# iSEE-Laboratory/DiffuVolume

Hardware: AMD Instinct MI355X
Metric: stereo pairs/sec, SceneFlow 960x540 (cropped 960x512) maxdisp=192, hot path (higher is better)
Workload: dtype f32; 1 GPU; SceneFlow ACVNet+DiffuVolume hot path (gwc + concat*softmax(att) + 5 DDIM steps + EPE), 960x512, maxdisp=192, batch=8/GPU, random-init weights; global_batch=8, ddim_steps=5, parallelism=dp1

## Files before the change

### diffuvolume_amd/_lib.py

```python
from __future__ import annotations

import ctypes
import os
from ctypes import POINTER, Structure, c_char_p, c_double, c_float, c_int, c_size_t, c_void_p
from pathlib import Path

import torch

_LIB_PATH = Path(os.environ.get("DV_LIB_PATH") or Path(__file__).resolve().parent / "libdiffuvolume_hip.so")
_lib = None


class DvDdimCoef(Structure):
    _fields_ = [("sqrt_recip_alpha", c_double), ("sqrt_recipm1_alpha", c_double),
                ("sqrt_alpha_next", c_double), ("c", c_double), ("sigma", c_double),
                ("dif_thr", c_float), ("unc_thr", c_float), ("cof", c_float), ("last", c_int),
                ("clamp_max", c_float), ("ens_dif_thr", c_float)]


P = c_void_p
I = c_int
SIGNATURES = {
    "dv_version": (c_int, []),
    "dv_error_string": (c_char_p, [I]),
# ... 4 lines not shown
    "dv_pointwise_expand_packed_floats": (c_size_t, [I, I]),
    "dv_pointwise_expand_pack_weights_f32": (c_int, [P, P, I, I, P]),
    "dv_pointwise_expand_f32": (c_int, [P, P, P, I, I, I, I, P]),
    "dv_softmax_d_f32": (c_int, [P, P, I, I, I, P]),
    "dv_mul_f32": (c_int, [P, P, P, c_size_t, P]),
    "dv_conv3d_rank1_filter_f32": (c_int, [P, P, P, P, P, P, I, I, I, I, I, I, P]),
    "dv_noise_prepare_f32": (c_int, [P, P, P, I, I, I, P]),
    "dv_noise_prepare_f64": (c_int, [P, P, P, P, I, I, I, P]),
    "dv_conv3d_packed_floats": (c_size_t, [I, I, I]),
    "dv_conv3d_pack_weights_f32": (c_int, [P, P, I, I, I, P]),
    "dv_conv3d_f32": (c_int, [P, P, P, P, P, P, P, I, I, I, I, I, I, I, I, I, P]),
    "dv_conv3d_set_s2_tile": (c_int, [I]),
    "dv_conv3d_set_c1z": (c_int, [I, I]),
    "dv_conv3d_f16x3_packed_bytes": (c_size_t, [I, I]),
    "dv_conv3d_f16x3_pack_weights": (c_int, [P, P, I, I, P]),
    "dv_conv3d_f16x3_f32": (c_int, [P, P, P, P, P, P, P, P, I, I, I, I, I, I, I, P]),
    "dv_conv3d_wino_packed_floats": (c_size_t, [I, I]),
    "dv_conv3d_wino_pack_weights_f32": (c_int, [P, P, I, I, P]),
    "dv_conv3d_wino_f32": (c_int, [P, P, P, P, P, P, P, I, I, I, I, I, I, I, P]),
    "dv_conv3d_wino3_packed_floats": (c_size_t, [I, I]),
    "dv_conv3d_wino3_supported": (c_int, [I, I, I, I, I]),
    "dv_conv3d_wino3_pack_weights_f32": (c_int, [P, P, I, I, P]),
    "dv_conv3d_wino3_f32": (c_int, [P, P, P, P, P, P, I, I, I, I, I, I, I, P]),
    "dv_conv3d_s2pp_supported": (c_int, [I, I, I, I, I]),
    "dv_conv3d_s2pp_packed_floats": (c_size_t, [I, I]),
    "dv_conv3d_s2pp_pack_weights_f32": (c_int, [P, P, I, I, P]),
    "dv_conv3d_s2pp_f32": (c_int, [P, P, P, P, P, P, I, I, I, I, I, I, I, P]),
    "dv_deconv3d_packed_floats": (c_size_t, [I, I]),
    "dv_deconv3d_pack_weights_f32": (c_int, [P, P, I, I, P]),
    "dv_deconv3d_k3s2_f32": (c_int, [P, P, P, P, P, P, I, I, I, I, I, I, I, P]),
    "dv_deconv3d_pl_supported": (c_int, [I, I, I, I, I, I]),
    "dv_deconv3d_set_impl": (c_int, [I]),
    "dv_deconv3d_pl_set_max_blocks": (c_int, [I]),
    "dv_deconv3d_k4_packed_floats": (c_size_t, [I, I]),
    "dv_deconv3d_k4_pack_weights_f32": (c_int, [P, P, I, I, P]),
    "dv_deconv3d_k4s2_f32": (c_int, [P, P, P, P, P, P, I, I, I, I, I, I, I, P]),
    "dv_conv2d_packed_floats": (c_size_t, [I, I, I, I]),
    "dv_conv2d_pack_weights_f32": (c_int, [P, P, I, I, I, I, P]),
    "dv_conv2d_f32": (c_int, [P, P, P, P, P, P, I, I, I, I, I, I, I, I, P]),
    "dv_conv2d_gated_f32": (c_int, [P, P, P, P, P, P, P, P, P, I, I, I, I, I, I, I, I, P]),
    "dv_conv2d_cat_f32": (c_int, [P, P, I, P, P, P, P, P, P, P, P, I, I, I, I, I, I, I, P]),
    "dv_conv2d_auto_kslices": (c_int, [I, I, I, I, I, I, I]),
    "dv_conv2d_cat_ksplit_f32": (c_int, [P, P, I, P, P, P, P, P, P, P, P, P, I, I, I, I, I, I, I, I, P]),
    "dv_conv2d_s2_f32": (c_int, [P, P, P, P, P, P, I, I, I, I, I, I, I, P]),
    "dv_conv2d_wino_packed_floats": (c_size_t, [I, I]),
    "dv_conv2d_wino_pack_weights_f32": (c_int, [P, P, I, I, P]),
    "dv_conv2d_wino_cat_f32": (c_int, [P, P, I, P, P, P, P, P, P, P, P, I, I, I, I, I, P]),
    "dv_conv2d_wino_cat_pair_f32": (c_int, [P, P, I, P, P, P, P, P, P, P, P, P, I, I, I, I, I, I, P]),
    "dv_conv2d_wino_dil_cat_f32": (c_int, [P, P, I, P, P, P, P, P, P, P, P, I, I, I, I, I, I, P]),
    "dv_refine_inputs_f32": (c_int, [P, P, P, P, P, P, I, I, I, I, I, P]),
    "dv_space_to_batch2_f32": (c_int, [P, P, I, I, I, I, P]),
    "dv_conv2d_wino_auto_kslices": (c_int, [I, I, I, I, I]),
    "dv_conv2d_wino_cat_ksplit_f32": (c_int, [P, P, I, P, P, P, P, P, P, P, P, P, I, I, I, I, I, I, I, P]),
    "dv_conv2d_wino_cat_pair_ksplit_f32": (c_int, [P, P, I, P, P, P, P, P, P, P, P, P, P, I, I, I, I, I, I, I, P]),
    "dv_conv2d_wino_s2b_f32": (c_int, [P, P, I, P, P, P, P, I, I, I, I, I, P]),
    "dv_batch_to_space_f32": (c_int, [P, P, I, I, I, I, I, P]),
    "dv_softmax_regress_f32": (c_int, [P, P, I, I, I, I, P]),
    "dv_feature_gate_f32": (c_int, [P, P, P, I, I, I, I, I, P]),
    "dv_deconv3d_k3s2_redir_f32": (c_int, [P, P, P, P, P, P, I, I, I, I, I, I, I, I, P]),
    "dv_patch_volume_f32": (c_int, [P, P, P, P, P, I, I, I, I, I, P]),
    "dv_patch_volume_runs_f32": (c_int, [P, P, P, P, P, I, I, I, I, I, I, P, P, P, P]),
    "dv_window_attn3d_f32": (c_int, [P, P, P, P, P, P, I, I, I, I, I, I, P]),
    "dv_upsample_softmax_regress_f32": (c_int, [P, P, P, I, I, I, I, I, P]),
    "dv_upsample_softmax_uncertainty_f32": (c_int, [P, P, P, I, I, I, I, I, P]),
    "dv_disparity_regression_f32": (c_int, [P, P, I, I, I, I, P]),
    "dv_encode_two_hot_f32": (c_int, [P, P, I, I, I, P]),
# ... 88 lines not shown
```

### diffuvolume_amd/csrc/deconv3d.hip

```cpp
#include <atomic>
#include <type_traits>

#include "dv_common.h"

int dv_deconv3d_pl_run(const float* in, const float* wpacked, const float* ch_scale, const float* ch_bias, const float* residual,
                       const float* skip, const float* rw, float* out, int B, int Cin, int D, int H, int W, int Cout, int Cskip,
                       int act, size_t wpk_floats, hipStream_t s);

namespace {

std::atomic<int> g_deconv_impl_pin{0};

typedef float f32x4 __attribute__((ext_vector_type(4)));

constexpr int kTD = 2, kTH = 2, kMTX = 2, kNT = 2;
constexpr int kTW = kMTX * 16;
constexpr int kCOUT = kNT * 16;

template <int K, int KC_>
struct DGeo {
  static constexpr int KC = KC_;
  static constexpr int LO = (K == 4) ? 1 : 0;
  static constexpr int T = K * K * K;
  static constexpr int IZ = kTD + 1 + LO, IY = kTH + 1 + LO, IX = kTW + 1 + LO;
  static constexpr int PRAW = IZ * IY * IX;
  static constexpr int P = PRAW + ((16 - PRAW % 32) + 32) % 32;
  static constexpr int IN_FLOATS = KC * P, W_FLOATS = T * KC * kCOUT;
  static_assert(P % 32 == 16, "bank rule");
  static_assert((IN_FLOATS + W_FLOATS) * 4 <= 80 * 1024, "two blocks per CU");
};
__host__ __device__ constexpr int tap_par(int k) { return (k + 1) & 1; }
__host__ __device__ constexpr int tap_off(int k) { return (k == 0 ? 1 : 0) - (k == 3 ? 1 : 0); }

struct DeconvArgs {
  const float* in;
  const float* wpk;
  const float* ch_scale;
  const float* ch_bias;
  const float* residual;
  const float* skip;
  const float* rw;
  int Cskip;
  float* out;
  int B, Cin, D, H, W, Cout, Coutp;
// ... 382 lines not shown
  if (blocks <= 0 || blocks > 0x7fffffffLL) return DV_ERR_SHAPE;
  hipLaunchKernelGGL((deconv3d_mfma_kernel<K, KC_>), dim3((unsigned)blocks), dim3(256), 0, s, a);
  return dv_launch_status();
}

constexpr int kc_of(int K) { return K == 3 ? 8 : 4; }

int pack_any(const float* w, float* wpacked, int Cin, int Cout, int K, hipStream_t s) {
  const int T = K * K * K, KC = kc_of(K), nchunk = pad_to(Cin, 8) / KC, nco = pad_to(Cout, kCOUT) / kCOUT;
  const size_t total = (size_t)nchunk * nco * T * KC * kCOUT;
  const int blocks = (int)((total + 255) / 256 < 4096 ? (total + 255) / 256 : 4096);
  hipLaunchKernelGGL(pack_deconv_weights_kernel, dim3(blocks), dim3(256), 0, s, w, wpacked, Cin, Cout, nchunk, nco, T, KC);
  return dv_launch_status();
}

int run_any(const float* in, const float* wpacked, const float* ch_scale, const float* ch_bias,
            const float* residual, float* out, int B, int Cin, int D, int H, int W, int Cout, int act, int K,
            hipStream_t s, const float* skip = nullptr, const float* rw = nullptr, int Cskip = 0) {
  DeconvArgs a;
  a.skip = skip; a.rw = rw; a.Cskip = Cskip;
  a.in = in; a.wpk = wpacked; a.ch_scale = ch_scale; a.ch_bias = ch_bias; a.residual = residual;
  a.out = out; a.B = B; a.Cin = Cin; a.D = D; a.H = H; a.W = W; a.Cout = Cout;
  a.Coutp = pad_to(Cout, kCOUT);
  a.ntx = (W + kTW - 1) / kTW;
  a.nty = (H + kTH - 1) / kTH;
  a.ntz = (D + kTD - 1) / kTD;
  a.nco = a.Coutp / kCOUT;
  a.act = act;
  a.vec_store = (W % 4 == 0) && dv_aligned16(out) && (!residual || dv_aligned16(residual));
  if ((size_t)D * H * W * sizeof(float) > 0x7fffffffull) return DV_ERR_SHAPE;
  a.fast_ok = (W % 2 == 0) && dv_aligned16(out) && (!residual || dv_aligned16(residual)) &&
              (size_t)Cout * 8 * D * H * W * sizeof(float) <= 0xffffffffull;
  const int pin = g_deconv_impl_pin.load(std::memory_order_relaxed);
  if (K == 3 && pin != 1 && (pin == 2 || !residual) &&
      dv_deconv3d_pl_supported(Cin, Cout, D, H, W, skip ? Cskip : 0) && dv_aligned16(in) && dv_aligned16(out) &&
      (!residual || dv_aligned16(residual)) && (!skip || dv_aligned16(skip)))
    return dv_deconv3d_pl_run(in, wpacked, ch_scale, ch_bias, residual, skip, rw, out, B, Cin, D, H, W, Cout, Cskip, act,
                              dv_deconv3d_packed_floats(Cin, Cout), s);
  return K == 3 ? launch_deconv<3, 8>(a, s) : launch_deconv<4, 4>(a, s);
}

}

extern "C" int dv_deconv3d_set_impl(int mode) {
  DV_REQUIRE(mode >= 0 && mode <= 2, DV_ERR_UNSUPPORTED);
  g_deconv_impl_pin.store(mode, std::memory_order_relaxed);
  return DV_OK;
}

extern "C" size_t dv_deconv3d_packed_floats(int Cin, int Cout) {
  if (Cin <= 0 || Cout <= 0) return 0;
  return (size_t)pad_to(Cin, 8) * 27 * pad_to(Cout, kCOUT);
}

extern "C" size_t dv_deconv3d_k4_packed_floats(int Cin, int Cout) {
  if (Cin <= 0 || Cout <= 0) return 0;
  return (size_t)pad_to(Cin, 8) * 64 * pad_to(Cout, kCOUT);
}

extern "C" int dv_deconv3d_pack_weights_f32(const float* w, float* wpacked, int Cin, int Cout, dv_stream_t stream) {
  DV_REQUIRE_PTR(w);
  DV_REQUIRE_PTR(wpacked);
  DV_REQUIRE(Cin > 0 && Cout > 0, DV_ERR_SHAPE);
  return pack_any(w, wpacked, Cin, Cout, 3, (hipStream_t)stream);
}

extern "C" int dv_deconv3d_k4_pack_weights_f32(const float* w, float* wpacked, int Cin, int Cout, dv_stream_t stream) {
  DV_REQUIRE_PTR(w);
  DV_REQUIRE_PTR(wpacked);
  DV_REQUIRE(Cin > 0 && Cout > 0, DV_ERR_SHAPE);
  return pack_any(w, wpacked, Cin, Cout, 4, (hipStream_t)stream);
}

#define DV_DECONV_CHECKS                                                             \
  DV_REQUIRE_PTR(in);                                                                \
  DV_REQUIRE_PTR(wpacked);                                                           \
  DV_REQUIRE_PTR(out);                                                               \
  DV_REQUIRE(B > 0 && Cin > 0 && D > 0 && H > 0 && W > 0 && Cout > 0, DV_ERR_SHAPE);  \
  DV_REQUIRE(act >= DV_ACT_NONE && act <= DV_ACT_LEAKY, DV_ERR_UNSUPPORTED);         \
  DV_REQUIRE(dv_aligned16(wpacked), DV_ERR_ALIGN);
// ... 31 lines not shown
```

### diffuvolume_amd/csrc/deconv3d_pl.hip

```cpp
#include <atomic>
#include <type_traits>

#include "dv_common.h"

namespace {

std::atomic<int> g_pl_max_blocks{0};

typedef float f32x4 __attribute__((ext_vector_type(4)));
typedef float f32x2 __attribute__((ext_vector_type(2)));
typedef int i32x4 __attribute__((ext_vector_type(4)));

namespace pl {
constexpr int TH = 2, TW = 32, KC = 8, NT = 2, COUT = 16 * NT;
constexpr int RQ = TW / 4 + 1;
constexpr int RS = 4 * RQ;
constexpr int IY = TH + 1, ROWS = 2 * IY;
constexpr int QPC = 60;
constexpr int CS = 4 * QPC;
static_assert(ROWS * RQ <= QPC && CS % 64 == 48, "brick image");
constexpr int BRICK_Q = KC * QPC;
constexpr int BRICK_P = (BRICK_Q + 63) / 64;
constexpr int BRICK_FLOATS = BRICK_P * 256;
constexpr int W_FLOATS = 27 * KC * COUT;
// ... 339 lines not shown

template <bool SKIP, bool RES, int AM>
int pl_launch(const PLArgs& a, hipStream_t s) {
  const int cap = g_pl_max_blocks.load(std::memory_order_relaxed);
  const long long slots = cap > 0 ? cap : pl_cu_count();
  const long long pairs = ((long long)a.nsp * a.nco + 1) / 2;
  const unsigned blocks = (unsigned)(pairs < slots ? pairs : slots);
  hipLaunchKernelGGL((deconv3d_pl_kernel<SKIP, RES, AM>), dim3(blocks), dim3(512 + 64 * pl::NL), 0, s, a);
  return dv_launch_status();
}

}

extern "C" int dv_deconv3d_pl_set_max_blocks(int n) {
  DV_REQUIRE(n >= 0, DV_ERR_SHAPE);
  g_pl_max_blocks.store(n, std::memory_order_relaxed);
  return DV_OK;
}

extern "C" int dv_deconv3d_pl_supported(int Cin, int Cout, int D, int H, int W, int Cskip) {
  if (Cin <= 0 || Cout <= 0 || D <= 0 || H <= 0 || W <= 0 || Cskip < 0) return 0;
  if (Cin % pl::KC || Cout % pl::COUT || Cout > pl::MAXCO || W % 4) return 0;
  if (Cskip % pl::SKC || Cskip / pl::SKC > Cin / pl::KC) return 0;
  const size_t vol = (size_t)D * H * W;
  if (vol * sizeof(float) * pl::KC > 0x7fffffffull) return 0;
  if ((size_t)Cout * 8 * vol * sizeof(float) > 0xffffffffull) return 0;
  if ((size_t)Cskip * 8 * vol * sizeof(float) > 0xffffffffull) return 0;
  return 1;
}

int dv_deconv3d_pl_run(const float* in, const float* wpacked, const float* ch_scale, const float* ch_bias, const float* residual,
                       const float* skip, const float* rw, float* out, int B, int Cin, int D, int H, int W, int Cout, int Cskip,
                       int act, size_t wpk_floats, hipStream_t s) {
  PLArgs a;
  a.in = in; a.wpk = wpacked; a.ch_scale = ch_scale; a.ch_bias = ch_bias; a.residual = residual; a.skip = skip; a.rw = rw;
  a.out = out; a.B = B; a.Cin = Cin; a.D = D; a.H = H; a.W = W; a.Cout = Cout; a.Cskip = skip ? Cskip : 0; a.act = act;
  a.ntx = pl_cdiv(W, pl::TW); a.nty = pl_cdiv(H, pl::TH); a.nco = Cout / pl::COUT;
  const long long tiles = (long long)B * D * a.nty * a.ntx;
  if (tiles <= 0 || tiles * a.nco > 0x3fffffffLL) return DV_ERR_SHAPE;
  a.nsp = (int)tiles;
  if (wpk_floats * sizeof(float) > 0x7fffffffull) return DV_ERR_SHAPE;
  a.wpk_bytes = (unsigned)(wpk_floats * sizeof(float));
  const int am = act == DV_ACT_RELU ? 0 : (act == DV_ACT_MISH ? 2 : 1);
  if (skip) {
    if (am == 0) return pl_launch<true, false, 0>(a, s);
    if (am == 2) return pl_launch<true, false, 2>(a, s);
    return pl_launch<true, false, 1>(a, s);
  }
  if (residual) {
    if (am == 0) return pl_launch<false, true, 0>(a, s);
    if (am == 2) return pl_launch<false, true, 2>(a, s);
    return pl_launch<false, true, 1>(a, s);
  }
  if (am == 0) return pl_launch<false, false, 0>(a, s);
  if (am == 2) return pl_launch<false, false, 2>(a, s);
  return pl_launch<false, false, 1>(a, s);
}
```

### diffuvolume_amd/submodule.py

```python
from __future__ import annotations

import ctypes
import itertools
import os
from typing import Optional, Tuple

import torch

from . import _lib
from .profiling import S2PP_MULT_REDUCTION, WINO3_MULT_REDUCTION, WINO_MULT_REDUCTION, timed

__all__ = ["build_gwc_volume", "build_concat_volume", "build_concat_attention_volume", "AttentionConcatVolume",
           "volume_factors",
           "disparity_regression", "upsample_softmax_regress", "Conv3dPlan", "Conv2dPlan", "Conv2dF16Plan", "Deconv3dPlan",
           "window_attention", "feature_gate", "softmax_regress", "refine_inputs", "patch_volume", "ACT_NONE", "ACT_RELU", "ACT_MISH", "ACT_LEAKY", "ACT_SIGMOID", "ACT_TANH"]

ACT_NONE, ACT_RELU, ACT_MISH, ACT_LEAKY, ACT_SIGMOID, ACT_TANH = 0, 1, 2, 3, 4, 5


_CONV_PRECISION = None


def set_default_conv_precision(precision=None) -> None:
    global _CONV_PRECISION
# ... 949 lines not shown
            self.cskip = rw.shape[1]
            rscale, rshift = _fold_bn(rbn, None, self.cout, w.device, redir_eps)
            one = torch.ones(self.cout, device=w.device)
            zero = torch.zeros(self.cout, device=w.device)
            sd, sr = (one if self.scale is None else self.scale), (one if rscale is None else rscale)
            w = w * sd.view(1, -1, 1, 1, 1)
            self.redir_w = (rw.reshape(self.cout, self.cskip) * sr.view(-1, 1)).contiguous()
            self.shift = ((zero if self.shift is None else self.shift) + (zero if rshift is None else rshift)).contiguous()
            self.scale = None
            self.redir_plan = Conv3dPlan(self.redir_w.view(self.cout, self.cskip, 1, 1, 1), None, stride=1, act=ACT_NONE,
                                         precision="f32")
        self.wpacked = torch.empty(sizer(self.cin, self.cout), dtype=torch.float32, device=w.device)
        with torch.cuda.device(w.device):
            _lib.check(packer(w.contiguous().data_ptr(), self.wpacked.data_ptr(), self.cin, self.cout, _lib.stream_ptr()),
                       "deconv weight packing")

    def __call__(self, x: torch.Tensor, residual: Optional[torch.Tensor] = None,
                 skip: Optional[torch.Tensor] = None) -> torch.Tensor:
        x = _dev_f32(x, "x")
        b, cin, d, h, w = x.shape
        if cin != self.cin:
            raise RuntimeError(f"expected {self.cin} input channels, got {cin}")
        out = torch.empty((b, self.cout, 2 * d, 2 * h, 2 * w), dtype=torch.float32, device=x.device)
        if skip is not None:
            if self.redir_w is None or residual is not None:
                raise RuntimeError("skip= needs a plan built with redir=, and excludes residual=")
            skip = _dev_f32(skip, "skip")
            if tuple(skip.shape) != (b, self.cskip, 2 * d, 2 * h, 2 * w):
                raise RuntimeError("skip shape mismatch")
            if w % 2 == 0 and (self.cskip + 7) // 8 <= (cin + 7) // 8:
                lib = _lib.load()
                with torch.cuda.device(x.device):
                    nb = 4.0 * (x.numel() + out.numel() + skip.numel())
                    timed("deconv3d_k3s2_redir", 2.0 * x.numel() * self.cout * 27 + 2.0 * out.numel() * self.cskip, nb,
                          lambda: _lib.check(lib.dv_deconv3d_k3s2_redir_f32(
                              x.data_ptr(), self.wpacked.data_ptr(), _lib.ptr(self.shift), skip.data_ptr(),
                              self.redir_w.data_ptr(), out.data_ptr(), b, cin, d, h, w, self.cout, self.cskip, self.act,
                              _lib.stream_ptr()), "dv_deconv3d_k3s2_redir_f32"), issued=2.0 * x.numel() * self.cout * 27 + 2.0 * out.numel() * self.cskip)
                return out
            residual = self.redir_plan(skip)
        if residual is not None:
            residual = _dev_f32(residual, "residual")
            if tuple(residual.shape) != tuple(out.shape):
                raise RuntimeError("residual shape mismatch")
        with torch.cuda.device(x.device):
            nb = 4.0 * (x.numel() + out.numel() * (1 if residual is None else 2))
            timed(f"deconv3d_k{self.k}s2", 2.0 * x.numel() * self.cout * self.k ** 3, nb,
                  lambda: _lib.check(self._run(x.data_ptr(), self.wpacked.data_ptr(), _lib.ptr(self.scale),
                                               _lib.ptr(self.shift), _lib.ptr(residual), out.data_ptr(), b, cin, d, h,
                                               w, self.cout, self.act, _lib.stream_ptr()), self._name), issued=2.0 * x.numel() * self.cout * self.k ** 3)
        return out


def _fold_bn(bn, bias, cout, device, eps):
    if bn is None and bias is None:
        return None, None
    if bn is None:
        return None, bias.detach().to(device=device, dtype=torch.float32).contiguous()
    gamma, beta, mean, var = (t.detach().to(device=device, dtype=torch.float32) for t in bn)
    scale = gamma / torch.sqrt(var + eps)
    shift = beta - mean * scale
    if bias is not None:
        shift = shift + bias.detach().to(device=device, dtype=torch.float32) * scale
    return scale.contiguous(), shift.contiguous()


def feature_gate(cv: torch.Tensor, logit: torch.Tensor, inplace: bool = False) -> torch.Tensor:
    cv = _dev_f32(cv, "cv")
    logit = _dev_f32(logit, "logit")
    b, c, d, h, w = cv.shape
    if tuple(logit.shape) != (b, c, h, w):
        raise RuntimeError(f"gate logits {tuple(logit.shape)} do not match volume {tuple(cv.shape)}")
    out = cv if inplace else torch.empty_like(cv)
    lib = _lib.load()
    with torch.cuda.device(cv.device):
        timed("feature_gate", float(cv.numel()), 8.0 * cv.numel(),
              lambda: _lib.check(lib.dv_feature_gate_f32(cv.data_ptr(), logit.data_ptr(), out.data_ptr(), b, c, d, h, w,
                                                         _lib.stream_ptr()), "dv_feature_gate_f32"))
    return out


def refine_inputs(left: torch.Tensor, right: torch.Tensor, disp: torch.Tensor, du_a: torch.Tensor,
                  du_b: torch.Tensor, maxshift: int = 24) -> torch.Tensor:
# ... 69 lines not shown
```

### include/diffuvolume_hip.h

```cpp
#ifndef DIFFUVOLUME_HIP_H
#define DIFFUVOLUME_HIP_H

#include <stddef.h>
#include <stdint.h>

#ifdef __cplusplus
extern "C" {
#endif

typedef void* dv_stream_t;

#define DV_OK 0
#define DV_ERR_NULL (-1)
#define DV_ERR_SHAPE (-2)
#define DV_ERR_UNSUPPORTED (-3)
#define DV_ERR_ALIGN (-4)

#define DV_ACT_NONE 0
#define DV_ACT_RELU 1
#define DV_ACT_MISH 2
#define DV_ACT_LEAKY 3
#define DV_ACT_SIGMOID 4
#define DV_ACT_TANH 5

// ... 47 lines not shown
size_t dv_conv3d_wino_packed_floats(int Cin, int Cout);
int dv_conv3d_wino_pack_weights_f32(const float* w , float* wpacked, int Cin, int Cout,
                                    dv_stream_t stream);
int dv_conv3d_wino_f32(const float* in, const float* wpacked, const float* ch_scale, const float* ch_bias,
                       const float* in_scale, const float* residual, float* out,
                       int B, int Cin, int D, int H, int W, int Cout, int act, dv_stream_t stream);

size_t dv_conv3d_wino3_packed_floats(int Cin, int Cout);
int dv_conv3d_wino3_supported(int Cin, int Cout, int D, int H, int W);
int dv_conv3d_wino3_pack_weights_f32(const float* w , float* wpacked, int Cin, int Cout,
                                     dv_stream_t stream);
int dv_conv3d_wino3_f32(const float* in, const float* wpacked, const float* ch_scale, const float* ch_bias,
                        const float* residual, float* out, int B, int Cin, int D, int H, int W, int Cout, int act,
                        dv_stream_t stream);

int dv_conv3d_s2pp_supported(int Cin, int Cout, int D, int H, int W);
size_t dv_conv3d_s2pp_packed_floats(int Cin, int Cout);
int dv_conv3d_s2pp_pack_weights_f32(const float* w , float* wpacked, int Cin, int Cout,
                                    dv_stream_t stream);
int dv_conv3d_s2pp_f32(const float* in, const float* wpacked, const float* ch_scale, const float* ch_bias,
                       const float* residual, float* out,
                       int B, int Cin, int D, int H, int W, int Cout, int act, dv_stream_t stream);

size_t dv_deconv3d_packed_floats(int Cin, int Cout);
int dv_deconv3d_pack_weights_f32(const float* w , float* wpacked,
                                 int Cin, int Cout, dv_stream_t stream);
int dv_deconv3d_k3s2_f32(const float* in, const float* wpacked, const float* ch_scale,
                         const float* ch_bias, const float* residual, float* out,
                         int B, int Cin, int D, int H, int W, int Cout, int act, dv_stream_t stream);

int dv_deconv3d_pl_supported(int Cin, int Cout, int D, int H, int W, int Cskip);
int dv_deconv3d_set_impl(int mode);
int dv_deconv3d_pl_set_max_blocks(int n);

size_t dv_deconv3d_k4_packed_floats(int Cin, int Cout);
int dv_deconv3d_k4_pack_weights_f32(const float* w , float* wpacked,
                                    int Cin, int Cout, dv_stream_t stream);
int dv_deconv3d_k4s2_f32(const float* in, const float* wpacked, const float* ch_scale,
                         const float* ch_bias, const float* residual, float* out,
                         int B, int Cin, int D, int H, int W, int Cout, int act, dv_stream_t stream);

size_t dv_conv2d_packed_floats(int Cin, int Cout, int k, int dilation);
int dv_conv2d_pack_weights_f32(const float* w, float* wpacked, int Cin, int Cout, int k, int dilation,
                               dv_stream_t stream);
int dv_conv2d_f32(const float* in, const float* wpacked, const float* ch_scale, const float* ch_bias,
                  const float* residual, float* out, int B, int Cin, int H, int W, int Cout, int k,
                  int dilation, int act, dv_stream_t stream);

int dv_conv2d_gated_f32(const float* in, const float* wpacked, const float* ch_scale, const float* ch_bias,
                        const float* residual, const float* mul, const float* blend_z, const float* blend_h,
                        float* out, int B, int Cin, int H, int W, int Cout, int k, int dilation, int act,
                        dv_stream_t stream);

int dv_conv2d_cat_f32(const float* const* inputs, const int* channels, int n_inputs, const float* wpacked,
                      const float* ch_scale, const float* ch_bias, const float* residual, const float* mul,
                      const float* blend_z, const float* blend_h, float* out, int B, int H, int W, int Cout,
                      int k, int dilation, int act, dv_stream_t stream);

int dv_conv2d_auto_kslices(int B, int Cin, int H, int W, int Cout, int k, int dilation);
int dv_conv2d_cat_ksplit_f32(const float* const* inputs, const int* channels, int n_inputs, const float* wpacked,
                             const float* ch_scale, const float* ch_bias, const float* residual, const float* mul,
                             const float* blend_z, const float* blend_h, float* out, float* scratch, int kslices,
                             int B, int H, int W, int Cout, int k, int dilation, int act, dv_stream_t stream);

int dv_conv2d_s2_f32(const float* in, const float* wpacked, const float* ch_scale, const float* ch_bias,
                     const float* residual, float* out, int B, int Cin, int H, int W, int Cout, int k, int act,
// ... 199 lines not shown
```

Before: 63.77 pairs/s.

## Add warp-specialized persistent deconv3d kernel with async LDS DMA producer waves

Adds a new persistent transposed-conv3d kernel in which dedicated producer waves stream input bricks and weights into LDS through buffer_load...lds DMA, while consumer waves run MFMA over output-pixel-pair tiles with a sub-pixel (parity) decomposition. This overlaps global loads with compute and skips the zero-stuffed taps. The kernel is routed by default only for the Cin=64, Cout=32, Cskip=32 shape, and the profiler's issued-FLOP accounting is adjusted to match. In exchange it adds a large, complex kernel with one block per CU and fixed tile assumptions.

```diff
diff --git a/diffuvolume_amd/_lib.py b/diffuvolume_amd/_lib.py
--- a/diffuvolume_amd/_lib.py
+++ b/diffuvolume_amd/_lib.py
@@ -60,6 +60,10 @@
     "dv_deconv3d_pl_supported": (c_int, [I, I, I, I, I, I]),
     "dv_deconv3d_set_impl": (c_int, [I]),
     "dv_deconv3d_pl_set_max_blocks": (c_int, [I]),
+    "dv_deconv3d_pp_supported": (c_int, [I, I, I, I, I, I]),
+    "dv_deconv3d_set_pp": (c_int, [I]),
+    "dv_deconv3d_pp_routed": (c_int, [I, I, I, I, I, I]),
+    "dv_deconv3d_pp_set_max_blocks": (c_int, [I]),
     "dv_deconv3d_k4_packed_floats": (c_size_t, [I, I]),
     "dv_deconv3d_k4_pack_weights_f32": (c_int, [P, P, I, I, P]),
     "dv_deconv3d_k4s2_f32": (c_int, [P, P, P, P, P, P, I, I, I, I, I, I, I, P]),
diff --git a/diffuvolume_amd/csrc/deconv3d.hip b/diffuvolume_amd/csrc/deconv3d.hip
--- a/diffuvolume_amd/csrc/deconv3d.hip
+++ b/diffuvolume_amd/csrc/deconv3d.hip
@@ -6,10 +6,26 @@
 int dv_deconv3d_pl_run(const float* in, const float* wpacked, const float* ch_scale, const float* ch_bias, const float* residual,
                        const float* skip, const float* rw, float* out, int B, int Cin, int D, int H, int W, int Cout, int Cskip,
                        int act, size_t wpk_floats, hipStream_t s);
+int dv_deconv3d_pp_run(const float* in, const float* wpacked, const float* ch_scale, const float* ch_bias, const float* residual,
+                       const float* skip, const float* rw, float* out, int B, int Cin, int D, int H, int W, int Cout, int Cskip,
+                       int act, size_t wpk_floats, hipStream_t s);
+extern "C" int dv_deconv3d_pp_supported(int Cin, int Cout, int D, int H, int W, int Cskip);
 
 namespace {
 
 std::atomic<int> g_deconv_impl_pin{0};
+std::atomic<int> g_deconv_pp_mode{0};
+
+bool pp_default(int Cin, int Cout, int Cskip) {
+  return Cin == 64 && Cout == 32 && Cskip == 32;
+}
+
+bool pp_routed(int Cin, int Cout, int D, int H, int W, int Cskip) {
+  const int mode = g_deconv_pp_mode.load(std::memory_order_relaxed);
+  if (g_deconv_impl_pin.load(std::memory_order_relaxed) != 0 || mode == 1) return false;
+  if (!dv_deconv3d_pp_supported(Cin, Cout, D, H, W, Cskip)) return false;
+  return mode == 2 || pp_default(Cin, Cout, Cskip);
+}
 
 typedef float f32x4 __attribute__((ext_vector_type(4)));
 
@@ -458,6 +474,10 @@
   a.fast_ok = (W % 2 == 0) && dv_aligned16(out) && (!residual || dv_aligned16(residual)) &&
               (size_t)Cout * 8 * D * H * W * sizeof(float) <= 0xffffffffull;
   const int pin = g_deconv_impl_pin.load(std::memory_order_relaxed);
+  if (K == 3 && !residual && pp_routed(Cin, Cout, D, H, W, skip ? Cskip : 0) && dv_aligned16(in) && dv_aligned16(out) &&
+      (!skip || dv_aligned16(skip)))
+    return dv_deconv3d_pp_run(in, wpacked, ch_scale, ch_bias, residual, skip, rw, out, B, Cin, D, H, W, Cout, Cskip, act,
+                              dv_deconv3d_packed_floats(Cin, Cout), s);
   if (K == 3 && pin != 1 && (pin == 2 || !residual) &&
       dv_deconv3d_pl_supported(Cin, Cout, D, H, W, skip ? Cskip : 0) && dv_aligned16(in) && dv_aligned16(out) &&
       (!residual || dv_aligned16(residual)) && (!skip || dv_aligned16(skip)))
@@ -472,6 +492,16 @@
   DV_REQUIRE(mode >= 0 && mode <= 2, DV_ERR_UNSUPPORTED);
   g_deconv_impl_pin.store(mode, std::memory_order_relaxed);
   return DV_OK;
+}
+
+extern "C" int dv_deconv3d_set_pp(int mode) {
+  DV_REQUIRE(mode >= 0 && mode <= 2, DV_ERR_UNSUPPORTED);
+  g_deconv_pp_mode.store(mode, std::memory_order_relaxed);
+  return DV_OK;
+}
+
+extern "C" int dv_deconv3d_pp_routed(int Cin, int Cout, int D, int H, int W, int Cskip) {
+  return pp_routed(Cin, Cout, D, H, W, Cskip) ? 1 : 0;
 }
 
 extern "C" size_t dv_deconv3d_packed_floats(int Cin, int Cout) {
diff --git a/diffuvolume_amd/csrc/deconv3d_pl.hip b/diffuvolume_amd/csrc/deconv3d_pl.hip
--- a/diffuvolume_amd/csrc/deconv3d_pl.hip
+++ b/diffuvolume_amd/csrc/deconv3d_pl.hip
@@ -395,6 +395,7 @@
 int dv_deconv3d_pl_run(const float* in, const float* wpacked, const float* ch_scale, const float* ch_bias, const float* residual,
                        const float* skip, const float* rw, float* out, int B, int Cin, int D, int H, int W, int Cout, int Cskip,
                        int act, size_t wpk_floats, hipStream_t s) {
+  if (skip && residual) return DV_ERR_UNSUPPORTED;
   PLArgs a;
   a.in = in; a.wpk = wpacked; a.ch_scale = ch_scale; a.ch_bias = ch_bias; a.residual = residual; a.skip = skip; a.rw = rw;
   a.out = out; a.B = B; a.Cin = Cin; a.D = D; a.H = H; a.W = W; a.Cout = Cout; a.Cskip = skip ? Cskip : 0; a.act = act;
diff --git a/diffuvolume_amd/csrc/deconv3d_pp.hip b/diffuvolume_amd/csrc/deconv3d_pp.hip
--- /dev/null
+++ b/diffuvolume_amd/csrc/deconv3d_pp.hip
@@ -0,0 +1,460 @@
+#include <atomic>
+#include <type_traits>
+
+#include "dv_common.h"
+
+namespace {
+
+std::atomic<int> g_pp_max_blocks{0};
+
+typedef float f32x4 __attribute__((ext_vector_type(4)));
+typedef float f32x2 __attribute__((ext_vector_type(2)));
+typedef int i32x4 __attribute__((ext_vector_type(4)));
+
+namespace pp {
+constexpr int TH = 4, TW = 32, KC = 8, COUT = 32;
+constexpr int RQ = TW / 4 + 1;
+constexpr int RS = 4 * RQ;
+constexpr int ROWS = TH + 1;
+constexpr int QPC = 56;
+constexpr int CS = 4 * QPC;
+static_assert(ROWS * RQ <= QPC && CS % 64 == 32, "brick image");
+constexpr int BRICK_Q = KC * QPC;
+constexpr int BRICK_P = BRICK_Q / 64;
+static_assert(BRICK_Q % 64 == 0, "brick in whole pieces");
+constexpr int BRICK_FLOATS = BRICK_P * 256;
+constexpr int W_FLOATS = 9 * KC * COUT;
+constexpr int W_P = W_FLOATS / 256;
+constexpr int SKC = 4;
+constexpr int SK_FLOATS = SKC * 4 * 2 * TW;
+constexpr int NL = 4;
+constexpr int OFF = 1;
+constexpr int NB = (BRICK_P + NL - 1) / NL, NW = (W_P + NL - 1) / NL;
+constexpr int MAXCO = 256;
+static_assert((4 * W_FLOATS + 4 * BRICK_FLOATS + 8 * SK_FLOATS + 2 * MAXCO) * 4 <= 160 * 1024, "one block per CU");
+}
+
+__device__ __forceinline__ void pp_dma16(i32x4 rsrc, unsigned lds, unsigned voff, unsigned soff) {
+  unsigned m0_saved;
+  asm volatile("s_mov_b32 %0, m0\n\ts_mov_b32 m0, %1\n\ts_nop 0\n\tbuffer_load_dwordx4 %2, %3, %4 offen lds\n\ts_mov_b32 m0, %0"
+               : "=&s"(m0_saved) : "s"(lds), "v"(voff), "s"(rsrc), "s"(soff) : "memory");
+}
+
+__host__ __device__ constexpr int pp_tsel(int a) { return a == 0 ? 0 : a == 1 ? 1 : a == 2 ? 2 : a == 3 ? 1 : 3; }
+__host__ __device__ constexpr int pp_wsel(int a) { return a <= 1 ? 0 : a - 1; }
+__host__ __device__ constexpr int pp_priv(int o) { return o == 0 ? 0 : o == 1 ? 2 : o == 2 ? 1 : 4; }
+
+struct PPArgs {
+  const float* in;
+  const float* wpk;
+  const float* ch_scale;
+  const float* ch_bias;
+  const float* skip;
+  const float* rw;
+  float* out;
+  int B, Cin, D, H, W, Cout, Cskip;
+  int ntx, nty, nco, nsp;
+  int act;
+  unsigned wpk_bytes;
+};
+
+struct PPTile { int tcb, xi, yi, z0, y0, x0, b; unsigned st; bool valid; };
+
+template <bool SKIP, int AM>
+__global__ __launch_bounds__(512 + 64 * pp::NL, 1) void deconv3d_pp_kernel(PPArgs a) {
+  using namespace pp;
+  __shared__ __attribute__((aligned(16))) float w_s[4][W_FLOATS];
+  __shared__ __attribute__((aligned(16))) float in_s[2][2][BRICK_FLOATS];
+  __shared__ __attribute__((aligned(16))) float sk_s[8][SK_FLOATS];
+  __shared__ __attribute__((aligned(16))) float sb_s[2][MAXCO];
+
+  const int tid = threadIdx.x, lane = tid & 63;
+  const int wave = __builtin_amdgcn_readfirstlane(tid >> 6);
+  for (int i = tid; i < a.Cout; i += 512 + 64 * NL) {
+    sb_s[0][i] = a.ch_scale ? a.ch_scale[i] : 1.f;
+    sb_s[1][i] = a.ch_bias ? a.ch_bias[i] : 0.f;
+  }
+
+  const unsigned nblk = gridDim.x, nx = nblk < 8u ? nblk : 8u, xcd = blockIdx.x % nx, bidx = blockIdx.x / nx;
+  const unsigned nbx = nblk / nx + (xcd < nblk % nx ? 1u : 0u);
+  const unsigned ntiles = (unsigned)a.nsp * (unsigned)a.nco;
+  const unsigned npairs = (ntiles + 1u) >> 1;
+  const unsigned tq = npairs / nx, trm = npairs % nx;
+  const unsigned slab_lo = xcd < trm ? xcd * (tq + 1) : trm * (tq + 1) + (xcd - trm) * tq;
+  const unsigned slab_n = tq + (xcd < trm ? 1u : 0u);
+  const int my_pairs = __builtin_amdgcn_readfirstlane(bidx < slab_n ? (int)((slab_n - bidx + nbx - 1) / nbx) : 0);
+  if (my_pairs == 0) return;
+  auto rfl = [](unsigned v) __attribute__((always_inline)) { return (unsigned)__builtin_amdgcn_readfirstlane((int)v); };
+  auto decode = [&](unsigned t, int (&d)[5]) __attribute__((always_inline)) {
+    d[0] = (int)rfl(t % a.nco); t /= a.nco;
+    d[1] = (int)rfl(t % a.ntx); t /= a.ntx;
+    d[2] = (int)rfl(t % a.nty); t /= a.nty;
+    d[3] = (int)rfl(t % a.D);
+    d[4] = (int)rfl(t / a.D);
+  };
+  int sd[5];
+  decode(2u * nbx, sd);
+  auto tile_first = [&](int g) __attribute__((always_inline)) {
+    PPTile r;
+    r.st = 2u * (slab_lo + bidx) + (unsigned)g;
+    r.valid = r.st < ntiles;
+    int d[5];
+    decode(r.valid ? r.st : ntiles - 1u, d);
+    r.tcb = d[0]; r.xi = d[1]; r.yi = d[2]; r.z0 = d[3]; r.b = d[4];
+    r.x0 = r.xi * TW; r.y0 = r.yi * TH;
+    return r;
+  };
+  auto tile_next = [&](PPTile& r) __attribute__((always_inline)) {
+    r.st += 2u * nbx;
+    r.valid = r.st < ntiles;
+    int c;
+    r.tcb += sd[0];      c = r.tcb >= a.nco; r.tcb -= c ? a.nco : 0;
+    r.xi += sd[1] + c;   c = r.xi >= a.ntx;  r.xi -= c ? a.ntx : 0;
+    r.yi += sd[2] + c;   c = r.yi >= a.nty;  r.yi -= c ? a.nty : 0;
+    r.z0 += sd[3] + c;   c = r.z0 >= a.D;    r.z0 -= c ? a.D : 0;
+    r.b += sd[4] + c;
+    r.x0 = r.xi * TW; r.y0 = r.yi * TH;
+  };
+
+  const size_t plane = (size_t)a.H * a.W, vol = (size_t)a.D * plane;
+  const unsigned vol_bytes = (unsigned)__builtin_amdgcn_readfirstlane((int)(vol * sizeof(float)));
+  const unsigned plane_bytes = (unsigned)__builtin_amdgcn_readfirstlane((int)(plane * sizeof(float)));
+  const int nchunk = a.Cin / KC;
+  const int PERIOD = 3 * nchunk + 2;
+  const int n_total = my_pairs * PERIOD + OFF;
+  auto phase = [&](int p, int& kz, int& c) __attribute__((always_inline)) {
+    if (p < nchunk) { kz = 1; c = p; return true; }
+    if (p == nchunk || p == PERIOD - 1) { kz = 1; c = 0; return false; }
+    if (p <= 2 * nchunk) { kz = 2; c = p - nchunk - 1; return true; }
+    kz = 0; c = p - 2 * nchunk - 1;
+    return true;
+  };
+  const bool shared = a.nco == 1;
+
+  if (wave >= 8) {
+    const int li = wave - 8;
+    const uint64_t wb = reinterpret_cast<uint64_t>(a.wpk);
+    const uint64_t wbs = (uint64_t)(unsigned)__builtin_amdgcn_readfirstlane((int)(unsigned)wb) |
+                         ((uint64_t)(unsigned)__builtin_amdgcn_readfirstlane((int)(unsigned)(wb >> 32)) << 32);
+    const auto wrs = __builtin_amdgcn_make_buffer_rsrc(reinterpret_cast<float*>(wbs), 0, (int)a.wpk_bytes, 0x00020000);
+    unsigned sob[2][NB];
+    auto plan = [&](const PPTile& t, unsigned (&so)[NB]) __attribute__((always_inline)) {
+#pragma unroll
+      for (int i = 0; i < NB; ++i) {
+        const int it = 64 * (li + NL * i) + lane;
+        const int cl = it / QPC, r1 = it - cl * QPC;
+        const int row = r1 / RQ, q = r1 - row * RQ;
+        const int y = t.y0 + row, x = t.x0 + 4 * q;
+        const bool ok = t.valid && it < BRICK_Q && row < ROWS && y < a.H && x < a.W;
+        so[i] = ok ? (unsigned)cl * vol_bytes + (unsigned)((t.z0 * a.H + y) * a.W + x) * 4u : 0xfffffff0u;
+      }
+    };
+    auto dma = [&](const PPTile& t, const unsigned (&so)[NB], int c, int kz, float* bdst, float* wdst, bool with_w) __attribute__((always_inline)) {
+      const uint64_t ba = reinterpret_cast<uint64_t>(a.in + ((size_t)t.b * a.Cin + (size_t)c * KC) * vol);
+      const uint64_t bu = (uint64_t)(unsigned)__builtin_amdgcn_readfirstlane((int)(unsigned)ba) |
+                          ((uint64_t)(unsigned)__builtin_amdgcn_readfirstlane((int)(unsigned)(ba >> 32)) << 32);
+      const auto rs = __builtin_amdgcn_make_buffer_rsrc(reinterpret_cast<float*>(bu), 0,
+                                                        __builtin_amdgcn_readfirstlane((int)((unsigned)KC * vol_bytes)), 0x00020000);
+      const bool up = kz == 0;
+      const bool dead = up && t.z0 + 1 >= a.D;
+#pragma unroll
+      for (int i = 0; i < NB; ++i)
+        if (li + NL * i < BRICK_P) {
+          const unsigned o = (dead || so[i] == 0xfffffff0u) ? 0xfffffff0u : so[i] + (up ? plane_bytes : 0u);
+          __builtin_amdgcn_raw_ptr_buffer_load_lds(rs, (__attribute__((address_space(3))) void*)(bdst + (li + NL * i) * 256), 16,
+                                                   (int)o, 0, 0, 0);
+        }
+      const int wbase = ((c * a.nco + t.tcb) * 27 + kz * 9) * 1024;
+#pragma unroll
+      for (int i = 0; i < NW; ++i)
+        if (with_w && li + NL * i < W_P)
+          __builtin_amdgcn_raw_ptr_buffer_load_lds(wrs, (__attribute__((address_space(3))) void*)(wdst + (li + NL * i) * 256), 16,
+                                                   lane * 16, wbase + (li + NL * i) * 1024, 0, 0);
+    };
+    PPTile ft[2] = {tile_first(0), tile_first(1)};
+    int fk[2] = {0, 0}, fp[2] = {0, 0}, fcc[2] = {0, 0};
+    plan(ft[0], sob[0]);
+    plan(ft[1], sob[1]);
+    auto prepare = [&](int s1) __attribute__((always_inline)) {
+#pragma unroll
+      for (int g = 0; g < 2; ++g) {
+        if (s1 < g * OFF || fk[g] >= my_pairs) continue;
+        int kz, c;
+        if (phase(fp[g], kz, c)) {
+          if (ft[g].valid) dma(ft[g], sob[g], c, kz, in_s[g][fcc[g] & 1], w_s[shared ? (fcc[g] & 3) : 2 * g + (fcc[g] & 1)], !shared || g == 0);
+          ++fcc[g];
+        }
+        if (++fp[g] == PERIOD) {
+          fp[g] = 0;
+          if (++fk[g] < my_pairs) { tile_next(ft[g]); plan(ft[g], sob[g]); }
+        }
+      }
+    };
+    prepare(0);
+    asm volatile("s_waitcnt vmcnt(0) lgkmcnt(0)\n\ts_barrier" ::: "memory");
+#pragma unroll 1
+    for (int s = 0; s < n_total; ++s) {
+      if (s + 1 < n_total) prepare(s + 1);
+      asm volatile("s_waitcnt vmcnt(0)\n\ts_barrier" ::: "memory");
+    }
+    return;
+  }
+
+  const int g = wave >> 2, yl = (wave >> 1) & 1, nh = wave & 1;
+  const int j = lane & 15, kq = lane >> 4;
+  float* const sk = sk_s[wave];
+  const int a_off = kq * CS + 2 * yl * RS + 2 * j;
+  const int Do = 2 * a.D, Ho = 2 * a.H, Wo = 2 * a.W;
+  const size_t oplane = (size_t)Ho * Wo, ovol = (size_t)Do * oplane;
+  const unsigned oplane_bytes = (unsigned)__builtin_amdgcn_readfirstlane((int)(unsigned)(oplane * sizeof(float)));
+  const unsigned ovol_bytes = (unsigned)__builtin_amdgcn_readfirstlane((int)(unsigned)(ovol * sizeof(float)));
+  const int nsk = SKIP ? a.Cskip / SKC : 0;
+
+  f32x4 acc[5][5];
+  auto zero_acc = [&]() __attribute__((always_inline)) {
+#pragma unroll
+    for (int ay = 0; ay < 5; ++ay)
+#pragma unroll
+      for (int ax = 0; ax < 5; ++ax) acc[ay][ax] = (f32x4){0.f, 0.f, 0.f, 0.f};
+  };
+
+  PPTile cur = tile_first(g);
+  unsigned skv = 0;
+  f32x4 sc4, bi4;
+  unsigned loff = 0;
+  int yi0 = 0;
+  bool row_ok0 = false, row_ok1 = false, x_ok = false;
+  auto tile_setup = [&]() __attribute__((always_inline)) {
+    yi0 = cur.y0 + 2 * yl;
+    row_ok0 = cur.valid && yi0 < a.H;
+    row_ok1 = cur.valid && yi0 + 1 < a.H;
+    x_ok = cur.x0 + 2 * j < a.W;
+    loff = (unsigned)(((size_t)(cur.tcb * COUT + nh * 16 + 4 * kq) * ovol + 2 * cur.x0 + 4 * j) * sizeof(float));
+    sc4 = *reinterpret_cast<const f32x4*>(&sb_s[0][cur.tcb * COUT + nh * 16 + 4 * kq]);
+    bi4 = *reinterpret_cast<const f32x4*>(&sb_s[1][cur.tcb * COUT + nh * 16 + 4 * kq]);
+    if (SKIP) {
+      const int row = lane >> 4, cq = lane & 15;
+      const int oy = 2 * yi0 + row, ox = 2 * cur.x0 + 4 * cq;
+      const bool ok = cur.valid && oy < Ho && ox < Wo;
+      skv = ok ? (unsigned)(((size_t)oy * Wo + ox) * sizeof(float)) : 0xfffffff0u;
+    }
+  };
+
+  auto compute = [&](bool sk_on, int c, int buf, int wslot, int oz) __attribute__((always_inline)) {
+    const bool has_sk = sk_on && c < nsk;
+    const float* ib = in_s[g][buf] + a_off;
+    const float* wl = w_s[wslot] + lane * 4 + nh;
+    float bw = 0.f;
+    if (SKIP) {
+      const uint64_t ba = reinterpret_cast<uint64_t>(a.skip + (size_t)cur.b * a.Cskip * ovol);
+      i32x4 rs;
+      rs[0] = __builtin_amdgcn_readfirstlane((int)(unsigned)ba);
+      rs[1] = __builtin_amdgcn_readfirstlane((int)(unsigned)(ba >> 32));
+      rs[2] = __builtin_amdgcn_readfirstlane((int)((unsigned)a.Cskip * ovol_bytes));
+      rs[3] = 0x00020000;
+      const unsigned skl = (unsigned)__builtin_amdgcn_readfirstlane((int)(unsigned)(uintptr_t)(__attribute__((address_space(3))) void*)sk);
+      const unsigned so = (unsigned)(c * SKC) * ovol_bytes + (unsigned)oz * oplane_bytes;
+      if (sk_on)
+#pragma unroll
+        for (int p = 0; p < SKC; ++p)
+          pp_dma16(rs, skl + p * 1024, has_sk ? skv : 0xfffffff0u, so + (unsigned)p * ovol_bytes);
+      bw = a.rw[(size_t)(cur.tcb * COUT + nh * 16 + j) * a.Cskip + (has_sk ? c : 0) * SKC + kq];
+    }
+    auto ldrow = [&](int r, float (&x)[3][2]) __attribute__((always_inline)) {
+#pragma unroll
+      for (int ks = 0; ks < 2; ++ks) {
+        const f32x2 lo = *reinterpret_cast<const f32x2*>(ib + ks * 4 * CS + r * RS);
+        const f32x2 hi = *reinterpret_cast<const f32x2*>(ib + ks * 4 * CS + r * RS + 2);
+        x[0][ks] = lo[0]; x[1][ks] = lo[1]; x[2][ks] = hi[0];
+      }
+    };
+    auto ldw = [&](int ky, float (&u)[4][2]) __attribute__((always_inline)) {
+#pragma unroll
+      for (int ks = 0; ks < 2; ++ks) {
+        const float t0 = wl[(ky * 3 + 0) * 256 + 2 * ks], t1 = wl[(ky * 3 + 1) * 256 + 2 * ks], t2 = wl[(ky * 3 + 2) * 256 + 2 * ks];
+        u[0][ks] = t1; u[1][ks] = t2; u[2][ks] = t2 + t0; u[3][ks] = t0;
+      }
+    };
+    auto colt = [&](const float (&x)[3][2], float (&t)[4][2]) __attribute__((always_inline)) {
+#pragma unroll
+      for (int ks = 0; ks < 2; ++ks) {
+        t[0][ks] = x[0][ks]; t[1][ks] = x[1][ks]; t[2][ks] = x[0][ks] - x[1][ks]; t[3][ks] = x[2][ks] - x[1][ks];
+      }
+    };
+    auto stage = [&](auto ayc, const float (&t)[4][2], const float (&w)[4][2]) __attribute__((always_inline)) {
+      constexpr int ay = decltype(ayc)::value;
+#pragma unroll
+      for (int ax = 0; ax < 5; ++ax)
+#pragma unroll
+        for (int ks = 0; ks < 2; ++ks)
+          acc[ay][ax] = __builtin_amdgcn_mfma_f32_16x16x4f32(w[pp_wsel(ax)][ks], t[pp_tsel(ax)][ks], acc[ay][ax], 0, 0, 0);
+    };
+    float r0[3][2], r1[3][2], r2[3][2], u0[4][2], u1[4][2], u2[4][2], t[4][2], d[3][2], us[4][2];
+    ldrow(0, r0); ldw(1, u1);
+    __builtin_amdgcn_sched_barrier(0);
+    ldrow(1, r1); ldw(2, u2);
+    colt(r0, t);
+    stage(std::integral_constant<int, 0>{}, t, u1);
+    __builtin_amdgcn_sched_barrier(0);
+#pragma unroll
+    for (int x = 0; x < 3; ++x)
+#pragma unroll
+      for (int ks = 0; ks < 2; ++ks) d[x][ks] = r0[x][ks] - r1[x][ks];
+    colt(d, t);
+    stage(std::integral_constant<int, 2>{}, t, u2);
+    __builtin_amdgcn_sched_barrier(0);
+    ldw(0, u0);
+    colt(r1, t);
+    stage(std::integral_constant<int, 1>{}, t, u1);
+    __builtin_amdgcn_sched_barrier(0);
+    ldrow(2, r2);
+#pragma unroll
+    for (int cx = 0; cx < 4; ++cx)
+#pragma unroll
+      for (int ks = 0; ks < 2; ++ks) us[cx][ks] = u2[cx][ks] + u0[cx][ks];
+    colt(r1, t);
+    stage(std::integral_constant<int, 3>{}, t, us);
+    __builtin_amdgcn_sched_barrier(0);
+#pragma unroll
+    for (int x = 0; x < 3; ++x)
+#pragma unroll
+      for (int ks = 0; ks < 2; ++ks) d[x][ks] = r2[x][ks] - r1[x][ks];
+    colt(d, t);
+    stage(std::integral_constant<int, 4>{}, t, u0);
+    __builtin_amdgcn_sched_barrier(0);
+    if (SKIP) {
+      asm volatile("s_waitcnt vmcnt(0)" ::: "memory");
+      asm volatile("" : "+v"(bw));
+    }
+    if (SKIP && sk_on) {
+      const float* skr = sk + kq * 256 + 4 * j;
+#pragma unroll
+      for (int r = 0; r < 4; ++r) {
+        const f32x4 sa = *reinterpret_cast<const f32x4*>(skr + r * 64);
+#pragma unroll
+        for (int ox = 0; ox < 4; ++ox)
+          acc[pp_priv(r)][pp_priv(ox)] = __builtin_amdgcn_mfma_f32_16x16x4f32(bw, sa[ox], acc[pp_priv(r)][pp_priv(ox)], 0, 0, 0);
+      }
+    }
+  };
+
+  const float slope = a.act == DV_ACT_LEAKY ? 0.01f : 1.f;
+  auto epilogue = [&](int oz) __attribute__((always_inline)) {
+    const size_t po = (size_t)cur.b * a.Cout * ovol + (size_t)oz * oplane;
+#pragma unroll
+    for (int o = 0; o < 4; ++o) {
+      if (!(o < 2 ? row_ok0 : row_ok1)) continue;
+      f32x4 rsum[5], v4[4];
+#pragma unroll
+      for (int ax = 0; ax < 5; ++ax)
+        rsum[ax] = o == 0 ? acc[0][ax] : o == 1 ? acc[2][ax] + acc[3][ax] : o == 2 ? acc[1][ax] : acc[3][ax] + acc[4][ax];
+      v4[0] = rsum[0]; v4[1] = rsum[2] + rsum[3]; v4[2] = rsum[1]; v4[3] = rsum[3] + rsum[4];
+      const size_t ro = po + (size_t)(2 * yi0 + o) * Wo;
+#pragma unroll
+      for (int e = 0; e < 4; ++e) {
+        char* orow = reinterpret_cast<char*>(a.out + ro + (size_t)e * ovol);
+        f32x4 v;
+#pragma unroll
+        for (int x = 0; x < 4; ++x) v[x] = fmaf(v4[x][e], sc4[e], bi4[e]);
+        if (AM == 0) {
+          v = __builtin_elementwise_max(v, v * 0.f);
+        } else {
+#pragma unroll
+          for (int x = 0; x < 4; ++x) v[x] = AM == 2 ? dv_act(v[x], DV_ACT_MISH) : fmaxf(v[x], v[x] * slope);
+        }
+        if (x_ok) *reinterpret_cast<f32x4*>(orow + loff) = v;
+      }
+    }
+  };
+
+  zero_acc();
+  int k = 0, p = 0, cc = 0;
+  asm volatile("s_waitcnt lgkmcnt(0)\n\ts_barrier" ::: "memory");
+  tile_setup();
+#pragma unroll 1
+  for (int s = 0; s < n_total; ++s) {
+    if (s >= g * OFF && k < my_pairs) {
+      int kz, c;
+      if (phase(p, kz, c)) {
+        const int wslot = shared ? (cc & 3) : 2 * g + (cc & 1);
+        if (cur.valid && !(kz == 0 && cur.z0 + 1 >= a.D)) {
+          compute(kz != 0, c, cc & 1, wslot, 2 * cur.z0 + (kz >> 1));
+        }
+        ++cc;
+      } else {
+        epilogue(2 * cur.z0 + (p == nchunk ? 0 : 1));
+        zero_acc();
+      }
+      if (++p == PERIOD) {
+        p = 0;
+        if (++k < my_pairs) { tile_next(cur); tile_setup(); }
+      }
+    }
+    asm volatile("s_waitcnt lgkmcnt(0)\n\ts_barrier" ::: "memory");
+  }
+}
+
+inline int pp_cdiv(int a, int b) { return (a + b - 1) / b; }
+
+int pp_cu_count() {
+  int dev = 0, v = 0;
+  if (hipGetDevice(&dev) != hipSuccess) return 256;
+  static std::atomic<int> cache[64];
+  if (dev >= 0 && dev < 64 && (v = cache[dev].load(std::memory_order_relaxed)) > 0) return v;
+  if (hipDeviceGetAttribute(&v, hipDeviceAttributeMultiprocessorCount, dev) != hipSuccess || v <= 0) return 256;
+  if (dev >= 0 && dev < 64) cache[dev].store(v, std::memory_order_relaxed);
+  return v;
+}
+
+template <bool SKIP, int AM>
+int pp_launch(const PPArgs& a, hipStream_t s) {
+  const int cap = g_pp_max_blocks.load(std::memory_order_relaxed);
+  const long long slots = cap > 0 ? cap : pp_cu_count();
+  const long long pairs = ((long long)a.nsp * a.nco + 1) / 2;
+  const unsigned blocks = (unsigned)(pairs < slots ? pairs : slots);
+  hipLaunchKernelGGL((deconv3d_pp_kernel<SKIP, AM>), dim3(blocks), dim3(512 + 64 * pp::NL), 0, s, a);
+  return dv_launch_status();
+}
+
+}
+
+extern "C" int dv_deconv3d_pp_set_max_blocks(int n) {
+  DV_REQUIRE(n >= 0, DV_ERR_SHAPE);
+  g_pp_max_blocks.store(n, std::memory_order_relaxed);
+  return DV_OK;
+}
+
+extern "C" int dv_deconv3d_pp_supported(int Cin, int Cout, int D, int H, int W, int Cskip) {
+  if (Cin <= 0 || Cout <= 0 || D <= 0 || H <= 0 || W <= 0 || Cskip < 0) return 0;
+  if (Cin % pp::KC || Cout % pp::COUT || Cout > pp::MAXCO || W % 4) return 0;
+  if (Cskip % pp::SKC || Cskip / pp::SKC > Cin / pp::KC) return 0;
+  const size_t vol = (size_t)D * H * W;
+  if (vol * sizeof(float) * pp::KC > 0x7fffffffull) return 0;
+  if ((size_t)Cout * 8 * vol * sizeof(float) > 0xffffffffull) return 0;
+  if ((size_t)Cskip * 8 * vol * sizeof(float) > 0xffffffffull) return 0;
+  return 1;
+}
+
+int dv_deconv3d_pp_run(const float* in, const float* wpacked, const float* ch_scale, const float* ch_bias, const float* residual,
+                       const float* skip, const float* rw, float* out, int B, int Cin, int D, int H, int W, int Cout, int Cskip,
+                       int act, size_t wpk_floats, hipStream_t s) {
+  if (residual) return DV_ERR_UNSUPPORTED;
+  PPArgs a;
+  a.in = in; a.wpk = wpacked; a.ch_scale = ch_scale; a.ch_bias = ch_bias; a.skip = skip; a.rw = rw;
+  a.out = out; a.B = B; a.Cin = Cin; a.D = D; a.H = H; a.W = W; a.Cout = Cout; a.Cskip = skip ? Cskip : 0; a.act = act;
+  a.ntx = pp_cdiv(W, pp::TW); a.nty = pp_cdiv(H, pp::TH); a.nco = Cout / pp::COUT;
+  const long long tiles = (long long)B * D * a.nty * a.ntx;
+  if (tiles <= 0 || tiles * a.nco > 0x3fffffffLL) return DV_ERR_SHAPE;
+  a.nsp = (int)tiles;
+  if (wpk_floats * sizeof(float) > 0x7fffffffull) return DV_ERR_SHAPE;
+  a.wpk_bytes = (unsigned)(wpk_floats * sizeof(float));
+  const int am = act == DV_ACT_RELU ? 0 : (act == DV_ACT_MISH ? 2 : 1);
+  if (skip) {
+    if (am == 0) return pp_launch<true, 0>(a, s);
+    if (am == 2) return pp_launch<true, 2>(a, s);
+    return pp_launch<true, 1>(a, s);
+  }
+  if (am == 0) return pp_launch<false, 0>(a, s);
+  if (am == 2) return pp_launch<false, 2>(a, s);
+  return pp_launch<false, 1>(a, s);
+}
diff --git a/diffuvolume_amd/submodule.py b/diffuvolume_amd/submodule.py
--- a/diffuvolume_amd/submodule.py
+++ b/diffuvolume_amd/submodule.py
@@ -1005,11 +1005,13 @@
                 lib = _lib.load()
                 with torch.cuda.device(x.device):
                     nb = 4.0 * (x.numel() + out.numel() + skip.numel())
-                    timed("deconv3d_k3s2_redir", 2.0 * x.numel() * self.cout * 27 + 2.0 * out.numel() * self.cskip, nb,
+                    dflop, rflop = 2.0 * x.numel() * self.cout * 27, 2.0 * out.numel() * self.cskip
+                    pp = lib.dv_deconv3d_pp_routed(cin, self.cout, d, h, w, self.cskip) == 1
+                    timed("deconv3d_k3s2_redir", dflop + rflop, nb,
                           lambda: _lib.check(lib.dv_deconv3d_k3s2_redir_f32(
                               x.data_ptr(), self.wpacked.data_ptr(), _lib.ptr(self.shift), skip.data_ptr(),
                               self.redir_w.data_ptr(), out.data_ptr(), b, cin, d, h, w, self.cout, self.cskip, self.act,
-                              _lib.stream_ptr()), "dv_deconv3d_k3s2_redir_f32"), issued=2.0 * x.numel() * self.cout * 27 + 2.0 * out.numel() * self.cskip)
+                              _lib.stream_ptr()), "dv_deconv3d_k3s2_redir_f32"), issued=(dflop / 1.44 if pp else dflop) + rflop)
                 return out
             residual = self.redir_plan(skip)
         if residual is not None:
@@ -1018,10 +1020,12 @@
                 raise RuntimeError("residual shape mismatch")
         with torch.cuda.device(x.device):
             nb = 4.0 * (x.numel() + out.numel() * (1 if residual is None else 2))
-            timed(f"deconv3d_k{self.k}s2", 2.0 * x.numel() * self.cout * self.k ** 3, nb,
+            dflop = 2.0 * x.numel() * self.cout * self.k ** 3
+            pp = self.k == 3 and residual is None and _lib.load().dv_deconv3d_pp_routed(cin, self.cout, d, h, w, 0) == 1
+            timed(f"deconv3d_k{self.k}s2", dflop, nb,
                   lambda: _lib.check(self._run(x.data_ptr(), self.wpacked.data_ptr(), _lib.ptr(self.scale),
                                                _lib.ptr(self.shift), _lib.ptr(residual), out.data_ptr(), b, cin, d, h,
-                                               w, self.cout, self.act, _lib.stream_ptr()), self._name), issued=2.0 * x.numel() * self.cout * self.k ** 3)
+                                               w, self.cout, self.act, _lib.stream_ptr()), self._name), issued=dflop / 1.44 if pp else dflop)
         return out
 
 
diff --git a/include/diffuvolume_hip.h b/include/diffuvolume_hip.h
--- a/include/diffuvolume_hip.h
+++ b/include/diffuvolume_hip.h
@@ -103,6 +103,11 @@
 int dv_deconv3d_pl_supported(int Cin, int Cout, int D, int H, int W, int Cskip);
 int dv_deconv3d_set_impl(int mode);
 int dv_deconv3d_pl_set_max_blocks(int n);
+
+int dv_deconv3d_pp_supported(int Cin, int Cout, int D, int H, int W, int Cskip);
+int dv_deconv3d_set_pp(int mode);
+int dv_deconv3d_pp_routed(int Cin, int Cout, int D, int H, int W, int Cskip);
+int dv_deconv3d_pp_set_max_blocks(int n);
 
 size_t dv_deconv3d_k4_packed_floats(int Cin, int Cout);
 int dv_deconv3d_k4_pack_weights_f32(const float* w , float* wpacked,
```

Result: no change. 64.08 pairs/s, median of 6 (+0.5%).
